# mcahny/vps

Measured on AMD Instinct MI355X. Metric: frames/sec FuseTrack 1024x2048, higher is better.
Workload: dtype f32-grade: f16x3 split operands (fp16 pair with scaled residual, 22 significand bits) on MFMA, f32 accumulate

## Files before the change

vps_amd/csrc/conv_h8p.hip:

```cpp
#include "conv_common.h"

namespace {

template <int N, typename F>
__device__ __forceinline__ void static_for_p(F&& f) {
    if constexpr (N > 0) {
        static_for_p<N - 1>(f);
        f(std::integral_constant<int, N - 1>{});
    }
}

template <int MODE, int KH, int KW>
__global__ __launch_bounds__(512, 2)
void conv_mfma_h8p_kernel(const vps_conv_desc d, const int tiles_m, const int tiles_n, const int chunks_per_split) {
    constexpr int TM = 2, TN = 2, WAVES_N = 2, BN = 128;
    constexpr int NTAP = KH * KW;
    static_assert(NTAP % 3 == 0 || NTAP == 4, "ring / register-set index of a tap must be static: 9 taps (9 % 3 == 0) or 4 taps (12-step cycle handled by the caller)");
    constexpr int HW = 32 + KW - 1, HH = 8 + KH - 1;
    constexpr int HROWS = HH * HW;
    constexpr int NLD = (HROWS + 63) / 64;
    typedef Split<MODE> SM;
    typedef typename SM::elem elem_t;
    typedef vec8<elem_t> x8;
    typedef vec4<elem_t> x4;
    constexpr int NSA = SM::NSA, NSB = SM::NSB, NLB = SM::NLB, NT = SM::NT;
    constexpr int PLANE = HROWS * LDS_LDH;
    constexpr int ABUF = NSA * PLANE;
    constexpr int NFRAG = NSB * 2 * (BN / 32);
    constexpr int BBUF = NFRAG * 512;
    static_assert(NFRAG * 64 == NSB * 512, "thread t stages chunk t of every plane");
    static_assert((2 * ABUF + 3 * BBUF) * 2 <= 160 * 1024, "LDS budget of the CU");

    __shared__ __attribute__((aligned(16))) elem_t As[2 * ABUF];
    __shared__ __attribute__((aligned(16))) elem_t Bs[3 * BBUF];

    const int t = threadIdx.x;
    int swz = xcd_swizzle(blockIdx.x, gridDim.x);
    int tile_n, tile_m, cls, split;
    decode_tile(d, swz, tiles_n, tiles_m, tile_n, tile_m, cls, split);

    const int py = cls / d.os_x, px = cls - py * d.os_x;
    const int H = d.H, W = d.W, cin_pad = d.cin_pad;
    const int tiles_x = (d.Qw + 31) >> 5, tiles_y = (d.Qh + 7) >> 3;
    const int tx = tile_m % tiles_x, tq = tile_m / tiles_x;
    const int ty = tq % tiles_y, n = tq / tiles_y;
    const int iy_org = ty * 8 - d.pad_y[py], ix_org = tx * 32 - d.pad_x[px];

    const int k4 = t & 7;
    const int r0 = t >> 3;
    const int chunk0 = split * chunks_per_split;
    const int nchunks = min(chunks_per_split, d.kpad / (BK * NTAP) - chunk0);
    const int nsteps = nchunks * NTAP;

    const int lane = t & 63;
    const int wave = __builtin_amdgcn_readfirstlane(t >> 6);
    const int wm = wave / WAVES_N, wn = wave - wm * WAVES_N;
    const int nbt = d.cout_pad >> 5, kst = d.kpad >> 4;
    const size_t wplane = (size_t)d.nclass * nbt * kst * 512;
    const __amdgpu_buffer_rsrc_t wrsrc = make_rsrc(d.w_split, (unsigned)(wplane * NSB * sizeof(elem_t)));
    const unsigned wbase = (unsigned)((((size_t)(cls * nbt + tile_n * (BN / 32)) * kst + 2 * (size_t)chunk0 * NTAP) * 512) * sizeof(elem_t));
    const __amdgpu_buffer_rsrc_t arsrc = make_rsrc(d.in, (unsigned)((size_t)d.N * H * W * d.in_ld * sizeof(float)));
    const unsigned ld4 = (unsigned)d.in_ld * 4u;

    f32x4 areg[NLD];
    int achunk = chunk0;
    x8 breg[3][NLB];
    float amax = 0.f;

    unsigned hoff[NLD];
#pragma unroll
    for (int i = 0; i < NLD; ++i) {
        const int hp = r0 + 64 * i;
        const int hy = hp / HW, hx = hp - hy * HW;
        const int iy = iy_org + hy, ix = ix_org + hx;
        const bool ok = hp < HROWS && (unsigned)iy < (unsigned)H && (unsigned)ix < (unsigned)W;
        hoff[i] = ok ? (unsigned)((n * H + iy) * W + ix) * ld4 + (unsigned)(d.in_coff + k4 * 4) * 4u : 0xFFFFFFF0u;
    }

    auto load_A = [&]() {
        const bool kv = achunk * BK + k4 * 4 < cin_pad;
        const unsigned coff = (unsigned)achunk * (BK * 4u);
        ++achunk;
#pragma unroll
        for (int i = 0; i < NLD; ++i)
            areg[i] = buffer_load16<f32x4>(arsrc, (kv && hoff[i] != 0xFFFFFFF0u) ? hoff[i] + coff : 0xFFFFFFF0u, 0u);
    };
    auto store_A = [&](const int i, const int buf) {
        x4 sp[NSA];
        split_act<MODE>(areg[i], sp, amax);
        const int row = r0 + 64 * i;
        if (row < HROWS) {
#pragma unroll
            for (int p = 0; p < NSA; ++p)
                *reinterpret_cast<x4*>(&As[buf * ABUF + p * PLANE + row * LDS_LDH + (((k4 >> 1) ^ lds_swz(row)) << 3) + ((k4 & 1) << 2)]) = sp[p];
        }
    };
    auto load_B = [&](const int step, const int set) {
        const int sc = min(step, nsteps - 1);
        const int f = wave, bcol = f % (BN / 32), slab = f / (BN / 32);
#pragma unroll
        for (int p = 0; p < NLB; ++p)
            breg[set][p] = buffer_load16<x8>(wrsrc, (unsigned)lane * 16u,
                                             wbase + (unsigned)(((size_t)p * wplane + ((size_t)bcol * kst + 2 * sc + slab) * 512) * sizeof(elem_t)));
    };
    auto store_B = [&](const int slot, const int set) {
#pragma unroll
        for (int p = 0; p < NLB; ++p) *reinterpret_cast<x8*>(&Bs[slot * BBUF + (t + 512 * p) * 8]) = breg[set][p];
        if constexpr (NLB < NSB) *reinterpret_cast<x8*>(&Bs[slot * BBUF + (t + 512 * NLB) * 8]) = derive_weight_plane<MODE>(breg[set][0]);
    };

    int hbase[TM];
#pragma unroll
    for (int a = 0; a < TM; ++a) hbase[a] = (wm * TM + a) * HW + (lane & 31);
    x8 af[2][NSA][TM];
    x8 bcur[2][NSB][TN];
    constexpr int NRD = NSA * TM + NSB * TN;
    auto read_frag = [&](const int j, const int m, const int abuf, const int toff, const int slot) {
        if (j < NSA * TM) {
            const int p = j / TM, a = j - p * TM;
            const int hrow = hbase[a] + toff;
            af[m][p][a] = *reinterpret_cast<const x8*>(&As[abuf * ABUF + p * PLANE + hrow * LDS_LDH + (((2 * m + (lane >> 5)) ^ lds_swz(hrow)) << 3)]);
        } else {
            const int jj = j - NSA * TM, p = jj / TN, b = jj - p * TN;
            bcur[m][p][b] = *reinterpret_cast<const x8*>(&Bs[slot * BBUF + (((p * 2 + m) * (BN / 32)) + wn * TN + b) * 512 + lane * 8]);
        }
    };

    f32x16 acc[TM][TN];
#pragma unroll
    for (int a = 0; a < TM; ++a)
#pragma unroll
        for (int b = 0; b < TN; ++b)
#pragma unroll
            for (int r = 0; r < 16; ++r) acc[a][b][r] = 0.f;

    load_A();
    load_B(0, 0);
    load_B(1, 1);
#pragma unroll
    for (int i = 0; i < NLD; ++i) store_A(i, 0);
    store_B(0, 0);
    store_B(1, 1);
    load_B(2, 2);
    load_A();
    __syncthreads();
#pragma unroll
    for (int j = 0; j < NRD; ++j) read_frag(j, 0, 0, 0, 0);

    constexpr int NMS = NT * TM * TN;
    constexpr int STG = NTAP / 2;
    constexpr int SPT = (NLD + STG - 1) / STG;
    auto mfma = [&](const int m, const int i) {
        const int q = i / (TM * TN), r = i - q * (TM * TN), a = r / TN, b = r - a * TN;
        acc[a][b] = split_mfma<MODE>(bcur[m][SM::PB[q]][b], af[m][SM::PA[q]][a], acc[a][b]);
    };

    auto tap = [&](const int chunk, auto tp_tag, auto r3_tag) {
        constexpr int tp = decltype(tp_tag)::value;
        constexpr int R3 = decltype(r3_tag)::value;
        const int cur = chunk & 1;
        const int step = chunk * NTAP + tp;
        constexpr int toff = (tp / KW) * HW + (tp % KW);
        constexpr int ntp = (tp + 1) % NTAP;
        constexpr int ntoff = (ntp / KW) * HW + (ntp % KW);
        const int nbuf = tp == NTAP - 1 ? cur ^ 1 : cur;
#pragma unroll
        for (int i = 0; i < NMS; ++i) {
            mfma(0, i);
            __builtin_amdgcn_sched_barrier(0);
            if (i == 0) load_B(step + 3, R3);
#pragma unroll
            for (int j = 0; j < NRD; ++j)
                if ((j * (NMS - 1)) / NRD + 1 == i || (NMS == 1 && i == 0)) read_frag(j, 1, cur, toff, R3);
            __builtin_amdgcn_sched_barrier(0);
        }
#pragma unroll
        for (int i = 0; i < NMS; ++i) {
            mfma(1, i);
            __builtin_amdgcn_sched_barrier(0);
            if (tp < STG) {
#pragma unroll
                for (int si = 0; si < SPT; ++si)
                    if (i == (si * NMS) / (SPT + 1) && tp * SPT + si < NLD) store_A(tp * SPT + si, cur ^ 1);
            }
            if (i == (SPT * NMS) / (SPT + 1)) {
                store_B((R3 + 2) % 3, (R3 + 2) % 3);
                if (tp == STG) load_A();
            }
#pragma unroll
            for (int j = 0; j < NRD; ++j)
                if ((j * (NMS - 1)) / NRD + 1 == i || (NMS == 1 && i == 0)) read_frag(j, 0, nbuf, ntoff, (R3 + 1) % 3);
            __builtin_amdgcn_sched_barrier(0);
        }
        __syncthreads();
    };

    if constexpr (NTAP % 3 == 0) {
        for (int chunk = 0; chunk < nchunks; ++chunk)
            static_for_p<NTAP>([&](auto tpc) {
                constexpr int TP = decltype(tpc)::value;
                tap(chunk, std::integral_constant<int, TP>{}, std::integral_constant<int, TP % 3>{});
            });
    } else {
        int chunk = 0;
        for (; chunk + 2 < nchunks; chunk += 3)
            static_for_p<3 * NTAP>([&](auto sc) {
                constexpr int S = decltype(sc)::value;
                tap(chunk + S / NTAP, std::integral_constant<int, S % NTAP>{}, std::integral_constant<int, S % 3>{});
            });
        if (chunk < nchunks) {
            static_for_p<NTAP>([&](auto sc) {
                constexpr int S = decltype(sc)::value;
                tap(chunk, std::integral_constant<int, S>{}, std::integral_constant<int, S % 3>{});
            });
            ++chunk;
            if (chunk < nchunks)
                static_for_p<NTAP>([&](auto sc) {
                    constexpr int S = decltype(sc)::value;
                    tap(chunk, std::integral_constant<int, S>{}, std::integral_constant<int, (NTAP + S) % 3>{});
                });
        }
    }
    report_range<MODE>(d, amax);
    conv_epilogue<TM, TN, BN, true, 5>(d, acc, tiles_m * 256, tile_m, tile_n, cls, split, py, px, wm, wn, lane, (cls * tiles_m + tile_m) * tiles_n + tile_n);
}

}

__attribute__((visibility("hidden")))
void vpsi_launch_conv_h8p(const vps_conv_desc& d, const conv_plan& p, hipStream_t s) {
    hipLaunchKernelGGL((conv_mfma_h8p_kernel<VPS_PREC_F16X3, 3, 3>), dim3(p.grid), dim3(p.block), 0, s, d, p.tiles_m, p.tiles_n, p.chunks_per_split);
}
```

vps_amd/csrc/conv_mfma.hip:

```cpp
#include "conv_common.h"

namespace {
template <int TM, int TN, int WAVES_M, int WAVES_N, bool DEFORM>
__global__ __launch_bounds__(256, 2)
void conv_mfma_f32_kernel(const vps_conv_desc d, const int M, const int tiles_m, const int tiles_n,
                          const int ksteps_per_split) {
    constexpr int BN = WAVES_N * TN * 32;
    static_assert(WAVES_M * TM * 32 == BM, "block M tile must be 128");
    static_assert(WAVES_M * WAVES_N == 4, "4 wavefronts per block");
    constexpr int NB = BN / 32;

    __shared__ __attribute__((aligned(16))) float As[BM * LDS_LD];
    __shared__ __attribute__((aligned(16))) float Bs[BN * LDS_LD];

    const int t = threadIdx.x;
    int swz = xcd_swizzle(blockIdx.x, gridDim.x);
    int tile_n, tile_m, cls, split;
    decode_tile(d, swz, tiles_n, tiles_m, tile_n, tile_m, cls, split);

    const int py = cls / d.os_x, px = cls - py * d.os_x;
    const int pad_y = d.pad_y[py], pad_x = d.pad_x[px];
    const float* __restrict__ wcls = d.w + (size_t)cls * d.cout_pad * d.kpad;

    const int H = d.H, W = d.W, KH = d.KH, KW = d.KW, cin_pad = d.cin_pad;
// ... 431 lines not shown
                            const int pos = ((w + 1) * NMF) / (NW + 1);
                            if (mf == (pos < 1 ? 1 : pos)) {
                                __builtin_amdgcn_sched_barrier(0);
                                work(w);
                                __builtin_amdgcn_sched_barrier(0);
                            }
                        }
                    }
        __syncthreads();
    };
    for (int step = 0; step < nsteps; step += 2) {
        kstep(step, std::integral_constant<int, 0>{});
        if (step + 1 < nsteps) kstep(step + 1, std::integral_constant<int, 1>{});
    }
    report_range<MODE>(d, amax);
    conv_epilogue<TM, TN, BN, false, 4, DEFORM>(d, acc, M, tile_m, tile_n, cls, split, py, px, wm, wn, lane, (cls * tiles_m + tile_m) * tiles_n + tile_n);
}

template <int TM, int TN, int WAVES_M, int WAVES_N, int MODE, int KH, int KW>
__global__ __launch_bounds__(256, 2)
void conv_mfma_bf16h_kernel(const vps_conv_desc d, const int tiles_m, const int tiles_n, const int chunks_per_split) {
    constexpr int BN = WAVES_N * TN * 32;
    static_assert(WAVES_M * TM * 32 == BM, "block M tile must be 128");
    static_assert(WAVES_M * WAVES_N == 4, "4 wavefronts per block");
    constexpr int NTAP = KH * KW;
    constexpr int HW = 16 + KW - 1, HH = 8 + KH - 1;
    constexpr int HROWS = HH * HW;
    constexpr int NLD = (HROWS + 31) / 32;
    typedef Split<MODE> SM;
    typedef typename SM::elem elem_t;
    typedef vec8<elem_t> x8;
    typedef vec4<elem_t> x4;
    constexpr int NSA = SM::NSA, NSB = SM::NSB;
    constexpr int PLANE = NLD * 32 * LDS_LDH;
    constexpr int ABUF = NSA * PLANE;

    __shared__ __attribute__((aligned(16))) elem_t As[2 * ABUF];

    const int t = threadIdx.x;
    int swz = xcd_swizzle(blockIdx.x, gridDim.x);
    int tile_n, tile_m, cls, split;
    decode_tile(d, swz, tiles_n, tiles_m, tile_n, tile_m, cls, split);

    const int py = cls / d.os_x, px = cls - py * d.os_x;
    const int H = d.H, W = d.W, cin_pad = d.cin_pad;
    const int tiles_x = (d.Qw + 15) >> 4, tiles_y = (d.Qh + 7) >> 3;
    const int tx = tile_m % tiles_x, tq = tile_m / tiles_x;
    const int ty = tq % tiles_y, n = tq / tiles_y;
    const int iy_org = ty * 8 - d.pad_y[py], ix_org = tx * 16 - d.pad_x[px];

    const int k4 = t & 7;
    const int r0 = t >> 3;
    const int chunk0 = split * chunks_per_split;
    const int nchunks = min(chunks_per_split, d.kpad / (BK * NTAP) - chunk0);
    const int nsteps = nchunks * NTAP;

    const int lane = t & 63;
    const int wave = __builtin_amdgcn_readfirstlane(t >> 6);
    const int wm = wave / WAVES_N, wn = wave - wm * WAVES_N;
    const int nbt = d.cout_pad >> 5, kst = d.kpad >> 4;
    const size_t wplane = (size_t)d.nclass * nbt * kst * 512;
    const __amdgpu_buffer_rsrc_t wrsrc = make_rsrc(d.w_split, (unsigned)(wplane * NSB * sizeof(elem_t)));
    const unsigned wbase = (unsigned)((((size_t)(cls * nbt + tile_n * (BN / 32) + wn * TN) * kst + 2 * (size_t)chunk0 * NTAP) * 512) * sizeof(elem_t));
    const unsigned wlane = (unsigned)lane * 16u;
    const __amdgpu_buffer_rsrc_t arsrc = make_rsrc(d.in, (unsigned)((size_t)d.N * H * W * d.in_ld * sizeof(float)));
    const unsigned ld4 = (unsigned)d.in_ld * 4u;

    f32x4 areg[NLD];
    int achunk = chunk0;
    x8 bnext[2][NSB][TN];
    float amax = 0.f;

    unsigned hoff[NLD];
#pragma unroll
    for (int i = 0; i < NLD; ++i) {
        const int hp = r0 + 32 * i;
        const int hy = hp / HW, hx = hp - hy * HW;
        const int iy = iy_org + hy, ix = ix_org + hx;
        const bool ok = hp < HROWS && (unsigned)iy < (unsigned)H && (unsigned)ix < (unsigned)W;
        hoff[i] = ok ? (unsigned)((n * H + iy) * W + ix) * ld4 + (unsigned)(d.in_coff + k4 * 4) * 4u : 0xFFFFFFF0u;
    }

    auto load_A = [&]() {
        const bool kv = achunk * BK + k4 * 4 < cin_pad;
        const unsigned coff = (unsigned)achunk * (BK * 4u);
        ++achunk;
#pragma unroll
        for (int i = 0; i < NLD; ++i)
            areg[i] = buffer_load16<f32x4>(arsrc, (kv && hoff[i] != 0xFFFFFFF0u) ? hoff[i] + coff : 0xFFFFFFF0u, 0u);
    };
    auto load_B = [&](int step, int m, int p) {
#pragma unroll
        for (int b = 0; b < TN; ++b)
            bnext[m][p][b] = buffer_load16<x8>(wrsrc, wlane, wbase + (unsigned)(((size_t)p * wplane + ((size_t)b * kst + 2 * step + m) * 512) * sizeof(elem_t)));
    };
    auto store_A = [&](int i, int buf) {
        x4 sp[NSA];
        split_act<MODE>(areg[i], sp, amax);
        const int row = r0 + 32 * i;
#pragma unroll
        for (int p = 0; p < NSA; ++p)
            *reinterpret_cast<x4*>(&As[buf * ABUF + p * PLANE + row * LDS_LDH + (((k4 >> 1) ^ lds_swz(row)) << 3) + ((k4 & 1) << 2)]) = sp[p];
    };

    int hbase[TM];
#pragma unroll
    for (int a = 0; a < TM; ++a) {
        const int j = wm * TM * 32 + a * 32 + (lane & 31);
        hbase[a] = (j >> 4) * HW + (j & 15);
    }
    x8 af[2][NSA][TM];
    auto read_A = [&](int m, int buf, int toff) {
#pragma unroll
        for (int a = 0; a < TM; ++a) {
            const int hrow = hbase[a] + toff;
            const int off = buf * ABUF + hrow * LDS_LDH + (((2 * m + (lane >> 5)) ^ lds_swz(hrow)) << 3);
#pragma unroll
            for (int p = 0; p < NSA; ++p) af[m][p][a] = *reinterpret_cast<const x8*>(&As[off + p * PLANE]);
        }
    };

    f32x16 acc[TM][TN];
#pragma unroll
    for (int a = 0; a < TM; ++a)
#pragma unroll
        for (int b = 0; b < TN; ++b)
#pragma unroll
            for (int r = 0; r < 16; ++r) acc[a][b][r] = 0.f;

    load_A();
#pragma unroll
    for (int m = 0; m < 2; ++m)
#pragma unroll
        for (int p = 0; p < NSB; ++p) load_B(0, m, p);
#pragma unroll
    for (int i = 0; i < NLD; ++i) store_A(i, 0);
    load_A();
    __syncthreads();

    constexpr int NT = SM::NT;
    constexpr int NMF = 2 * NT * TM * TN;
    constexpr int SPT = (NLD + NTAP - 2) / (NTAP - 1);

    for (int chunk = 0; chunk < nchunks; ++chunk) {
        const int cur = chunk & 1;
#pragma unroll
        for (int tp = 0; tp < NTAP; ++tp) {
            const int step = chunk * NTAP + tp;
            const int bstep = min(step + 1, nsteps - 1);
            const int toff = (tp / KW) * HW + (tp % KW);
            constexpr int NLB = NSB;
            x8 bcur[2][NSB][TN];
#pragma unroll
            for (int m = 0; m < 2; ++m) {
#pragma unroll
                for (int p = 0; p < NLB; ++p)
#pragma unroll
                    for (int b = 0; b < TN; ++b) bcur[m][p][b] = bnext[m][p][b];
                if constexpr (NLB < NSB) {
#pragma unroll
                    for (int b = 0; b < TN; ++b) bcur[m][2][b] = derive_weight_plane<MODE>(bcur[m][0][b]);
                }
            }
            read_A(0, cur, toff);
            __builtin_amdgcn_sched_barrier(0);

            const int NW = SPT + 1 + 2 * NLB;
            auto work = [&](const int w) {
                if (w == 1) read_A(1, cur, toff);
                else if (w == 0 || (w >= 2 && w < SPT + 1)) {
                    const int si = (w == 0 ? 0 : w - 1);
                    if (tp < NTAP - 1) {
                        const int row = tp * SPT + si;
                        if (row < NLD) store_A(row, cur ^ 1);
                    } else if (si == 0) load_A();
                } else load_B(bstep, (w - SPT - 1) / NLB, (w - SPT - 1) % NLB);
            };

            int mf = 0;
#pragma unroll
            for (int m = 0; m < 2; ++m)
#pragma unroll
                for (int q = 0; q < NT; ++q)
#pragma unroll
                    for (int a = 0; a < TM; ++a)
#pragma unroll
                        for (int b = 0; b < TN; ++b) {
                            acc[a][b] = split_mfma<MODE>(bcur[m][SM::PB[q]][b], af[m][SM::PA[q]][a], acc[a][b]);
                            ++mf;
#pragma unroll
                            for (int w = 0; w < NW; ++w) {
                                const int pos = ((w + 1) * NMF) / (NW + 1);
                                if (mf == (pos < 1 ? 1 : pos)) {
                                    __builtin_amdgcn_sched_barrier(0);
                                    work(w);
                                    __builtin_amdgcn_sched_barrier(0);
                                }
                            }
                        }
        }
        __syncthreads();
    }
    report_range<MODE>(d, amax);
    conv_epilogue<TM, TN, BN, true>(d, acc, tiles_m * BM, tile_m, tile_n, cls, split, py, px, wm, wn, lane, (cls * tiles_m + tile_m) * tiles_n + tile_n);
}

template <int V>
__global__ __launch_bounds__(256)
void conv_splitk_reduce_kernel(const vps_conv_desc d, const int M) {
    const int cv = d.cout / V;
    const size_t total = (size_t)d.nclass * M * cv;
    const size_t plane = (size_t)d.nclass * M * d.cout_pad;
    for (size_t idx = (size_t)blockIdx.x * blockDim.x + threadIdx.x; idx < total;
         idx += (size_t)gridDim.x * blockDim.x) {
        const int co = (int)(idx % cv) * V;
        const size_t t2 = idx / cv;
        const int m = (int)(t2 % M);
        const int cls = (int)(t2 / M);
        const float* __restrict__ wp = d.ws + ((size_t)cls * M + m) * d.cout_pad + co;
        float s[V];
#pragma unroll
        for (int e = 0; e < V; ++e) s[e] = 0.f;
        for (int sp0 = 0; sp0 < d.ksplit; sp0 += 8) {
            float v[8][V];
#pragma unroll
            for (int j = 0; j < 8; ++j) {
                const float* q = wp + (size_t)min(sp0 + j, d.ksplit - 1) * plane;
                if constexpr (V == 4) {
                    const f32x4 t = *reinterpret_cast<const f32x4*>(q);
                    v[j][0] = t[0]; v[j][1] = t[1]; v[j][2] = t[2]; v[j][3] = t[3];
                } else {
                    v[j][0] = q[0];
                }
            }
#pragma unroll
            for (int j = 0; j < 8; ++j)
#pragma unroll
                for (int e = 0; e < V; ++e) s[e] = (sp0 + j < d.ksplit) ? s[e] + v[j][e] : s[e];
        }
        const int py = cls / d.os_x, px = cls - py * d.os_x;
        const int qx = m % d.Qw;
        const int tq = m / d.Qw;
        const int qy = tq % d.Qh;
        const int n = tq / d.Qh;
        const int oy = qy * d.os_y + py, ox = qx * d.os_x + px;
        const size_t opix = ((size_t)n * d.Ho + oy) * d.Wo + ox;
        const int rs = d.res_shift;
        const size_t rpix = ((size_t)n * (d.Ho >> rs) + (oy >> rs)) * (d.Wo >> rs) + (ox >> rs);
        float r[V];
#pragma unroll
        for (int e = 0; e < V; ++e) r[e] = 0.f;
        if (d.res) {
            if constexpr (V == 4) {
                const f32x4 t = *reinterpret_cast<const f32x4*>(d.res + rpix * d.res_ld + d.res_coff + co);
                r[0] = t[0]; r[1] = t[1]; r[2] = t[2]; r[3] = t[3];
            } else {
                r[0] = d.res[rpix * d.res_ld + d.res_coff + co];
            }
        }
        float o[V];
#pragma unroll
        for (int e = 0; e < V; ++e) {
            float v = s[e] * (d.scale ? d.scale[co + e] : 1.f) + (d.shift ? d.shift[co + e] : 0.f);
            if (d.res) v += r[e];
            o[e] = vps_act(v, d.act, d.slope);
        }
        float* op = d.out + opix * d.out_ld + d.out_coff + co;
        if constexpr (V == 4) *reinterpret_cast<f32x4*>(op) = f32x4{o[0], o[1], o[2], o[3]};
        else op[0] = o[0];
    }
}

template <int TM, int TN, int WAVES_M, int WAVES_N>
void launch_conv(const vps_conv_desc& d, const conv_plan& p, hipStream_t s) {
    const dim3 grid(p.grid), block(p.block);
    if (p.kernel == CONV_K_HALO) {
        with_prec<true>(d.prec, [&](auto mode) {
            constexpr int MODE = decltype(mode)::value;
            if (d.KH == 3) hipLaunchKernelGGL((conv_mfma_bf16h_kernel<TM, TN, WAVES_M, WAVES_N, MODE, 3, 3>), grid, block, 0, s, d, p.tiles_m, p.tiles_n, p.chunks_per_split);
            else hipLaunchKernelGGL((conv_mfma_bf16h_kernel<TM, TN, WAVES_M, WAVES_N, MODE, 2, 2>), grid, block, 0, s, d, p.tiles_m, p.tiles_n, p.chunks_per_split);
        });
        return;
    }
#define VPS_CONV_LAUNCH(KERNEL) hipLaunchKernelGGL((KERNEL), grid, block, 0, s, d, p.M, p.tiles_m, p.tiles_n, p.per_split)
    if (p.kernel == CONV_K_F32) {
        if (d.offset) VPS_CONV_LAUNCH((conv_mfma_f32_kernel<TM, TN, WAVES_M, WAVES_N, true>));
        else VPS_CONV_LAUNCH((conv_mfma_f32_kernel<TM, TN, WAVES_M, WAVES_N, false>));
        return;
    }
    const bool tapmajor = d.korder == 0 && d.KH * d.KW > 1;
    with_prec<true>(d.prec, [&](auto mode) {
        constexpr int MODE = decltype(mode)::value;
        if (d.offset) VPS_CONV_LAUNCH((conv_mfma_bf16p_kernel<TM, TN, WAVES_M, WAVES_N, MODE, false, true>));
        else if (tapmajor) VPS_CONV_LAUNCH((conv_mfma_bf16p_kernel<TM, TN, WAVES_M, WAVES_N, MODE, true>));
        else VPS_CONV_LAUNCH((conv_mfma_bf16p_kernel<TM, TN, WAVES_M, WAVES_N, MODE, false>));
    });
#undef VPS_CONV_LAUNCH
}

conv_switches conv_switches_now(const vps_conv_desc& d) {
    const auto on = [](const char* name) { const char* const e = getenv(name); return !(e && atoi(e) == 0); };
    const auto not0 = [](const char* name) { const char* const e = getenv(name); return !(e && e[0] == '0'); };
    static const bool s2_halo = not0("VPS_S2_HALO"), thin = on("VPS_THIN"), debug_occ = getenv("VPS_DEBUG_OCC") != nullptr;
    conv_switches sw = {true, true, true, true, s2_halo, thin, debug_occ};
    if (d.prec != VPS_PREC_F16X3) return sw;
    if (d.tile_n == 32) {
        if (d.cout > 16) sw.n32 = not0("VPS_N32");
        else if (d.nclass == 4) sw.n16t = on("VPS_N16T");
    } else if (d.tile_n <= 128 && d.KH == 1) sw.pw = on("VPS_PW");
    else if (d.tile_n == 128 && d.KH == 3 && d.stride == 1) sw.h8p = on("VPS_H8P");
    return sw;
}

const conv_limits& conv_limits_once(const bool debug) {
    static const conv_limits lim = [debug] {
        conv_limits l = {};
        int dev = 0;
        (void)hipGetDevice(&dev);
        (void)hipDeviceGetAttribute(&l.cus, hipDeviceAttributeMultiprocessorCount, dev);
        vpsi_conv_pw_limits(l, debug);
        vpsi_conv_thin_limits(l, debug);
        if (debug) vpsi_conv_q_debug_occ();
        return l;
    }();
    return lim;
}

}

extern "C" int vps_conv2d(const vps_conv_desc* dp, void* stream) {
    if (!dp) return VPS_EARG(1);
    const vps_conv_desc& d = *dp;
    if (const int e = vpsi_conv_check(d)) return e;
    const conv_switches sw = conv_switches_now(d);
    const conv_plan p = vpsi_conv_plan(d, conv_limits_once(sw.debug_occ), sw);
    hipStream_t s = (hipStream_t)stream;
    switch (p.kernel) {
        case CONV_K_NONE: return p.err;
        case CONV_K_SMALL3X3V: case CONV_K_SMALL_BATCHED: case CONV_K_SMALL: vpsi_launch_conv_small(d, p, s); break;
        case CONV_K_THIN: vpsi_launch_conv_thin(d, p, s); break;
        case CONV_K_DCN256:
            hipLaunchKernelGGL((conv_mfma_bf16p_kernel<2, 4, 2, 2, VPS_PREC_F16X3, false, true>), dim3(p.grid), dim3(p.block), 0, s, d, p.M, p.tiles_m, p.tiles_n, p.per_split);
            break;
        case CONV_K_N16T: case CONV_K_N32: case CONV_K_N16: vpsi_launch_conv_n16(d, p, s); break;
        case CONV_K_H8S2: vpsi_launch_conv_h8s2(d, p, s); break;
        case CONV_K_H8P: vpsi_launch_conv_h8p(d, p, s); break;
        case CONV_K_H8: vpsi_launch_conv_h8(d, p, s); break;
        case CONV_K_PW: vpsi_launch_conv_pw(d, p, s); break;
        case CONV_K_Q: vpsi_launch_conv_q(d, p, s); break;
        default:
            if (d.tile_n == 128) launch_conv<2, 2, 2, 2>(d, p, s);
            else if (d.tile_n == 64) launch_conv<2, 1, 2, 2>(d, p, s);
            else launch_conv<1, 1, 4, 1>(d, p, s);
    }
    int st = vps_launch_status();
    if (st || !p.needs_reduce) return st;
    const size_t total = (size_t)d.nclass * p.M * d.cout;
    if (p.reduce_v4) hipLaunchKernelGGL(conv_splitk_reduce_kernel<4>, dim3(stream_grid((long)(total / 4), 256)), dim3(256), 0, s, d, p.M);
    else hipLaunchKernelGGL(conv_splitk_reduce_kernel<1>, dim3(stream_grid((long)total, 256)), dim3(256), 0, s, d, p.M);
    return vps_launch_status();
}
```

vps_amd/csrc/conv_plan.cpp:

```cpp
#include "conv_plan.h"
#include <stdint.h>

namespace {

constexpr int BM = 128, BK = 32;

inline int cdiv(long a, long b) { return (int)((a + b - 1) / b); }
inline size_t in_bytes(const vps_conv_desc& d) { return (size_t)d.N * d.H * d.W * d.in_ld * sizeof(float); }
inline size_t out_bytes(const vps_conv_desc& d) { return (size_t)d.N * d.Ho * d.Wo * d.out_ld * sizeof(float); }
inline bool two_plane(int prec) { return prec == VPS_PREC_F16X3 || prec == VPS_PREC_BF16X3 || prec == VPS_PREC_BF16; }

constexpr int H8_MIN_CHUNKS = 3;
constexpr int PW_MIN_ROUNDS = 2;

conv_plan fail(conv_plan p, int n) { p.kernel = CONV_K_NONE; p.err = VPS_EARG(n); return p; }

conv_plan plan_small(const vps_conv_desc& d, conv_plan p) {
    p.block = 256;
    p.G = 1; p.logG = 0;
    while (p.G < 64 && p.G < (d.cin_pad >> 2)) { p.G <<= 1; ++p.logG; }
    const size_t wbytes = (size_t)(d.cout <= 2 ? 2 : 4) * d.kpad * sizeof(float);
    if (d.KH == 3 && d.KW == 3 && d.stride == 1 && d.nclass == 1 && d.pad_y[0] == 1 && d.pad_x[0] == 1 && d.Ho == d.H && d.Wo == d.W &&
        wbytes <= 150 * 1024 && (d.cout <= 2 || d.cout_pad >= 4) && in_bytes(d) < 0xFFFFFFF0ull &&
        (long)d.N * d.H * d.W < 0x7fffffffL) {
        const int run = d.cout <= 2 ? 4 : 2;
        p.runs_per_row = (d.W + run - 1) / run;
        const long total_runs = (long)d.N * d.H * p.runs_per_row;
        const int ppw = 64 >> p.logG;
        long blocks = (total_runs + 4 * ppw - 1) / (4 * ppw);
        if (blocks > 768) blocks = 768;
        p.kernel = CONV_K_SMALL3X3V; p.total_runs = (int)total_runs; p.grid = (unsigned)blocks; p.smem = wbytes;
        return p;
    }
    const long total = (long)d.nclass * p.M;
    const size_t wb = (size_t)d.nclass * (d.cout <= 2 ? 2 : 4) * d.kpad * sizeof(float);
    if ((d.cin_pad >> 2) * d.KH * d.KW >= 8 && wb <= 48 * 1024 && (d.cout <= 2 || d.cout_pad >= 4) && in_bytes(d) < 0xFFFFFFF0ull) {
        const int c4n = d.cin_pad >> 2, ntap = d.KH * d.KW;
        p.G = 1; p.logG = 0;
        while (p.G < 64 && p.G * 8 < c4n * ntap && p.G < c4n) { p.G <<= 1; ++p.logG; }
        p.nslot = (c4n + p.G - 1) >> p.logG;
        const int ppw = 64 >> p.logG;
        const long waves = (total + ppw - 1) / ppw;
        long blocks = (waves + 3) / 4; if (blocks > 2048) blocks = 2048; if (blocks < 1) blocks = 1;
        p.kernel = CONV_K_SMALL_BATCHED; p.grid = (unsigned)blocks; p.smem = wb;
        return p;
    }
    const long waves = (total + (64 >> p.logG) - 1) / (64 >> p.logG);
    long blocks = (waves + 3) / 4; if (blocks > 8192) blocks = 8192; if (blocks < 1) blocks = 1;
    p.kernel = CONV_K_SMALL; p.grid = (unsigned)blocks;
    return p;
}

bool plan_thin(const vps_conv_desc& d, const conv_limits& lim, const conv_switches& sw, conv_plan& p) {
    if (!sw.thin || !d.w_thin || d.prec != VPS_PREC_F16X3 || d.offset || d.res || d.nclass != 1 || d.ksplit != 1 || d.korder != 0) return false;
    if (d.KH != d.KW || d.cout_pad != 64 || d.tile_n != 64 || (d.cout & 3) || ((uintptr_t)d.w_thin & 15)) return false;
    if (d.pad_y[0] != d.KH / 2 || d.pad_x[0] != d.KH / 2 || d.pad_y[1] != d.KH / 2 || d.pad_x[1] != d.KH / 2) return false;
    if (in_bytes(d) >= 0xFFFFFFF0ull) return false;
    if (((d.out_ld | d.out_coff) & 3) || ((uintptr_t)d.out & 15) || out_bytes(d) >= 0xFFFFFFF0ull) return false;
    int i = 0;
    while (i < 4 && !(d.KH == conv_thin_shapes[i].ks && d.stride == conv_thin_shapes[i].s && d.cin_pad == conv_thin_shapes[i].c4)) ++i;
    if (i == 4) return false;
    const int ph = conv_thin_shapes[i].ph;
    const int tiles_x = (d.Qw + 31) / 32, tiles_y = (d.Qh + ph - 1) / ph;
    const long ntiles = (long)d.N * tiles_x * tiles_y;
    if (ntiles < 512 || ntiles > 0x7fffffffL) return false;
    const int resident = (lim.thin_per_cu[i] > 0 ? lim.thin_per_cu[i] : 1) * (lim.cus > 0 ? lim.cus : 256);
    const long rounds = (ntiles + resident - 1) / resident;
    p.kernel = CONV_K_THIN; p.thin = i; p.tiles_n = tiles_x; p.tiles_m = tiles_y; p.ntiles = (int)ntiles;
    p.grid = (unsigned)((ntiles + rounds - 1) / rounds); p.block = 256;
    return true;
}

bool plan_pw(const vps_conv_desc& d, const conv_limits& lim, const conv_switches& sw, conv_plan& p) {
    if (!sw.pw || d.prec != VPS_PREC_F16X3 || d.offset || d.KH != 1 || d.KW != 1 || d.nclass != 1 || d.ksplit != 1 || d.gn_stats) return false;
    if (d.pad_y[0] || d.pad_x[0] || (d.cin_pad & 31) || d.kpad != d.cin_pad || (d.tile_n != 128 && d.tile_n != 64)) return false;
    const int nk = d.kpad / BK;
    if (nk < 2 || (nk & 1)) return false;
    if (d.Ho != d.Qh || d.Wo != d.Qw || (d.stride == 1 && (d.H != d.Qh || d.W != d.Qw))) return false;
    if (((d.cout | d.out_ld | d.out_coff) & 3) || ((uintptr_t)d.out & 15) || out_bytes(d) >= 0xFFFFFE00ull) return false;
    if (d.res && (((d.res_ld | d.res_coff) & 3) || ((uintptr_t)d.res & 15) || d.res_shift < 0 || d.res_shift > 4 ||
                  (size_t)d.N * (d.Ho >> d.res_shift) * (d.Wo >> d.res_shift) * d.res_ld * sizeof(float) >= 0xFFFFFE00ull)) return false;
    if (in_bytes(d) >= 0xFFFFFE00ull) return false;
    const int per_cu = lim.pw_per_cu[d.tile_n == 128 ? 1 : 0];
    const int resident = (per_cu > 0 ? per_cu : 1) * (lim.cus > 0 ? lim.cus : 256);
    const long total = (long)p.tiles_m * p.tiles_n;
    const int unit = 8 * p.tiles_n;
    if (resident < unit || total < (long)PW_MIN_ROUNDS * resident) return false;
    const long rounds = (total + resident - 1) / resident;
    long grid = (total + rounds - 1) / rounds;
    grid = (grid + unit - 1) / unit * unit;
    if (grid > resident) grid = resident / unit * unit;
    const int mper = (int)(grid / unit);
    p.kernel = CONV_K_PW; p.grid = (unsigned)grid; p.nk = nk; p.nit = (p.tiles_m + mper * 8 - 1) / (mper * 8);
    return true;
}

}

const conv_thin_shape conv_thin_shapes[4] = {{8, 3, 1, 8}, {12, 3, 1, 8}, {4, 7, 2, 8}, {12, 7, 2, 4}};

const char* vpsi_conv_kernel_name(int kernel) {
    static const char* const names[] = {"none", "small3x3v", "small_batched", "small", "thin", "dcn256", "n16t", "n32", "n16",
                                        "h8s2", "h8p", "h8", "halo", "pw", "q", "f32", "bf16p"};
    return kernel >= 0 && kernel <= CONV_K_BF16P ? names[kernel] : "?";
}

int vpsi_conv_check(const vps_conv_desc& d) {
    if (!d.in || !d.out) return VPS_EARG(2);
    if (d.prec < VPS_PREC_F32 || d.prec > VPS_PREC_F16X3) return VPS_EARG(12);
    if (d.prec == VPS_PREC_F32 ? !d.w : !d.w_split) return VPS_EARG(13);
    if ((d.in_ld & 3) || (d.in_coff & 3) || (d.cin_pad & 3) || d.cin_pad <= 0) return VPS_EARG(3);
    if ((d.kpad % BK) || d.kpad < d.KH * d.KW * d.cin_pad || (d.korder != 0 && d.korder != 1)) return VPS_EARG(4);
    if (d.korder == 1 && d.kpad != d.KH * d.KW * ((d.cin_pad + BK - 1) / BK) * BK) return VPS_EARG(14);
    if (d.tile_n != 32 && d.tile_n != 64 && d.tile_n != 128 && !(d.tile_n == 256 && d.offset && d.prec == VPS_PREC_F16X3 && d.korder == 1)) return VPS_EARG(5);
    if (d.cout_pad % d.tile_n || d.cout > d.cout_pad || d.cout <= 0) return VPS_EARG(6);
    if (d.nclass != d.os_y * d.os_x || d.nclass < 1 || d.os_y > 2 || d.os_x > 2) return VPS_EARG(7);
    if (d.ksplit < 1 || (d.ksplit > 1 && !d.ws)) return VPS_EARG(8);
    if (d.offset && (d.nclass != 1 || d.off_ld < 2 * d.KH * d.KW || d.KH * d.KW > 9 || d.H > 65535 || d.W > 65535)) return VPS_EARG(9);
    if (d.offset && d.prec != VPS_PREC_F32 && d.korder != 1) return VPS_EARG(17);
    if (((uintptr_t)d.in & 15) || ((uintptr_t)d.w & 15) || ((uintptr_t)d.w_split & 15)) return VPS_EARG(10);
    if (d.prec != VPS_PREC_F32 && in_bytes(d) >= 0xFFFFFFF0ull) return VPS_EARG(16);
    if (d.gn_stats && (!d.offset || d.prec == VPS_PREC_F32 || d.ksplit != 1 || d.gn_rep < 1 || (d.gn_rep & (d.gn_rep - 1)) || (d.gn_cpg != 4 && (d.gn_cpg < 8 || (d.gn_cpg & 7))) || d.cout % d.gn_cpg ||
                       ((d.cout | d.out_ld | d.out_coff) & 3) || ((uintptr_t)d.out & 15) || d.res || ((uintptr_t)d.gn_stats & 7)))
        return VPS_EARG(15);
    const long Ml = (long)d.N * d.Qh * d.Qw;
    if (Ml <= 0 || Ml > 0x7fffffffL) return VPS_EARG(11);
    return 0;
}

conv_plan vpsi_conv_plan(const vps_conv_desc& d, const conv_limits& lim, const conv_switches& sw) {
    conv_plan p = {};
    const int M = p.M = (int)((long)d.N * d.Qh * d.Qw);
    if (d.cout <= 4 && d.prec == VPS_PREC_F32 && !d.offset && d.ksplit == 1 && d.tile_n == 32) return plan_small(d, p);
    if (plan_thin(d, lim, sw, p)) return p;

    const int BN = d.tile_n;
    const int tiles_m = p.tiles_m = cdiv(M, BM);
    const int tiles_n = p.tiles_n = d.cout_pad / BN;
    const int ksteps = d.kpad / BK;
    p.block = 256;
    p.needs_reduce = d.ksplit > 1 && !d.tile_counter;
    if (BN == 256) {
        p.per_split = cdiv(ksteps, d.ksplit);
        if (cdiv(ksteps, p.per_split) != d.ksplit) return fail(p, 20);
        p.kernel = CONV_K_DCN256; p.grid = (unsigned)((long)tiles_m * tiles_n * d.ksplit); p.reduce_v4 = true;
        return p;
    }
    const int ntap = d.KH * d.KW;
    const int nch = d.korder == 1 ? ksteps / ntap : 0;
    const bool chunk_split = d.ksplit > 1 && d.korder == 1 && nch > 0 && cdiv(nch, cdiv(nch, d.ksplit)) == d.ksplit;
    const int per_split = p.per_split = chunk_split ? cdiv(nch, d.ksplit) * ntap : cdiv(ksteps, d.ksplit);
    p.chunks_per_split = per_split / ntap;
    if (cdiv(ksteps, per_split) != d.ksplit) return fail(p, 20);
    const long nblk = (long)tiles_m * tiles_n * d.nclass * d.ksplit;
    if (nblk <= 0 || nblk > 0x7fffffffL) return fail(p, 21);
    p.reduce_v4 = !((d.cout | d.cout_pad | d.out_ld | d.out_coff) & 3) && !((uintptr_t)d.out & 15) &&
                  (!d.res || (!((d.res_ld | d.res_coff) & 3) && !((uintptr_t)d.res & 15)));
    const long tiles2d = (long)d.N * ((d.Qh + 7) / 8) * ((d.Qw + 15) / 16);
    const bool halo = d.prec != VPS_PREC_F32 && !d.offset && d.stride == 1 && d.korder == 1 && d.KH == d.KW && (d.KH == 3 || d.KH == 2) &&
                      tiles2d * 128 * 2 <= (long)M * 3 && (d.ksplit == 1 || chunk_split);
    const long tiles2d8 = (long)d.N * ((d.Qh + 7) / 8) * ((d.Qw + 31) / 32);
    const bool h8 = halo && BN == 128 && two_plane(d.prec) && tiles2d8 * 256 * 2 <= (long)M * 3 &&
                    tiles2d8 * tiles_n * d.nclass * d.ksplit >= 256 && ksteps / ntap >= H8_MIN_CHUNKS;
    const bool h8s2 = sw.s2_halo && (BN == 128 || BN == 64) && two_plane(d.prec) && !d.offset &&
                      d.stride == 2 && d.nclass == 1 && d.korder == 1 && d.KH == d.KW && (d.KH == 3 || d.KH == 5) &&
                      d.pad_y[0] == d.KH / 2 && d.pad_x[0] == d.KW / 2 && tiles2d8 * 256 * 2 <= (long)M * 3 &&
                      tiles2d8 * tiles_n * d.ksplit >= 256 && (d.ksplit == 1 || chunk_split);
    const bool n16 = BN == 32 && d.prec == VPS_PREC_F16X3 && halo && d.cout > 4 && d.cout <= (sw.n32 ? 32 : 16) && d.cout_pad == 32 && d.ksplit == 1 &&
                     !d.gn_stats && tiles2d8 * 256 * 2 <= (long)M * 3 && tiles2d8 * d.nclass >= 256;
    if (n16) {
        const bool fused = sw.n16t && d.KH == 2 && d.KW == 2 && d.nclass == 4 && d.os_y == 2 && d.os_x == 2 &&
                           d.pad_y[0] >= 0 && d.pad_y[0] <= 1 && d.pad_y[1] >= 0 && d.pad_y[1] <= 1 &&
                           d.pad_x[0] >= 0 && d.pad_x[0] <= 1 && d.pad_x[1] >= 0 && d.pad_x[1] <= 1;
        p.tiles_m = (int)tiles2d8; p.block = 512;
        if (fused && d.cout <= 16) { p.kernel = CONV_K_N16T; p.grid = (unsigned)tiles2d8; }
        else { p.kernel = d.cout > 16 ? CONV_K_N32 : CONV_K_N16; p.grid = (unsigned)(tiles2d8 * d.nclass); }
    } else if (h8s2) {
        p.kernel = CONV_K_H8S2; p.tiles_m = (int)tiles2d8; p.block = 512; p.grid = (unsigned)(tiles2d8 * tiles_n * d.ksplit);
    } else if (h8) {
        p.kernel = sw.h8p && d.prec == VPS_PREC_F16X3 && d.KH == 3 ? CONV_K_H8P : CONV_K_H8;
        p.tiles_m = (int)tiles2d8; p.block = 512; p.grid = (unsigned)(tiles2d8 * tiles_n * d.nclass * d.ksplit);
    } else if (halo) {
        const long nblk2 = tiles2d * tiles_n * d.nclass * d.ksplit;
        if (nblk2 > 0x7fffffffL) return fail(p, 21);
        p.kernel = CONV_K_HALO; p.tiles_m = (int)tiles2d; p.grid = (unsigned)nblk2;
    } else {
        p.grid = (unsigned)nblk;
        const bool tapmajor = d.korder == 0 && ntap > 1;
        const bool q_ok = BN >= 64 && !tapmajor;
        if (q_ok && plan_pw(d, lim, sw, p)) return p;
        if (q_ok && !d.offset && two_plane(d.prec)) p.kernel = CONV_K_Q;
        else p.kernel = d.prec == VPS_PREC_F32 ? CONV_K_F32 : CONV_K_BF16P;
    }
    return p;
}
```

vps_amd/csrc/conv_plan.h:

```cpp
#pragma once
#include <stddef.h>
#include "../../include/vps_hip.h"

#ifndef VPS_EARG
#define VPS_EARG(x) (-1000 - (x))
#endif

enum conv_kernel {
    CONV_K_NONE = 0,
    CONV_K_SMALL3X3V,
    CONV_K_SMALL_BATCHED,
    CONV_K_SMALL,
    CONV_K_THIN,
    CONV_K_DCN256,
    CONV_K_N16T,
    CONV_K_N32,
    CONV_K_N16,
    CONV_K_H8S2,
    CONV_K_H8P,
    CONV_K_H8,
    CONV_K_HALO,
    CONV_K_PW,
    CONV_K_Q,
    CONV_K_F32,
    CONV_K_BF16P,
};

struct conv_plan {
    int kernel;
    int err;
    int M;
    int tiles_m, tiles_n;
    int per_split;
    int chunks_per_split;
    unsigned grid, block;
    size_t smem;
    int nk, nit;
    int G, logG, nslot;
    int runs_per_row, total_runs;
    int thin;
    int ntiles;
    bool needs_reduce;
    bool reduce_v4;
};

struct conv_limits {
    int cus;
    int pw_per_cu[2];
    int thin_per_cu[4];
};

struct conv_switches {
    bool pw;
    bool h8p;
    bool n16t;
    bool n32;
    bool s2_halo;
    bool thin;
    bool debug_occ;
};

struct conv_thin_shape { int c4, ks, s, ph; };
extern const conv_thin_shape conv_thin_shapes[4];

int vpsi_conv_check(const vps_conv_desc& d);
conv_plan vpsi_conv_plan(const vps_conv_desc& d, const conv_limits& lim, const conv_switches& sw);
const char* vpsi_conv_kernel_name(int kernel);

#ifdef __HIPCC__
void vpsi_launch_conv_small(const vps_conv_desc& d, const conv_plan& p, hipStream_t s);
void vpsi_launch_conv_thin(const vps_conv_desc& d, const conv_plan& p, hipStream_t s);
void vpsi_launch_conv_n16(const vps_conv_desc& d, const conv_plan& p, hipStream_t s);
void vpsi_launch_conv_h8(const vps_conv_desc& d, const conv_plan& p, hipStream_t s);
void vpsi_launch_conv_h8p(const vps_conv_desc& d, const conv_plan& p, hipStream_t s);
void vpsi_launch_conv_h8s2(const vps_conv_desc& d, const conv_plan& p, hipStream_t s);
void vpsi_launch_conv_pw(const vps_conv_desc& d, const conv_plan& p, hipStream_t s);
void vpsi_launch_conv_q(const vps_conv_desc& d, const conv_plan& p, hipStream_t s);
void vpsi_conv_pw_limits(conv_limits& lim, bool debug);
void vpsi_conv_thin_limits(conv_limits& lim, bool debug);
void vpsi_conv_q_debug_occ();
#endif
```

Baseline: 56.91.

## Add wide 256-column h8 halo conv kernel with per-slab pipelined refills

Adds a 3x3 stride-1 f16x3 convolution kernel that covers 256 output channels per block instead of 128. Each halo activation tile loaded into LDS is therefore reused across twice as many output columns, reducing activation traffic and split work per FLOP. Each tap is split into two half-slabs, and weight loads, LDS stores and fragment reads are interleaved between MFMAs on a three-slot weight ring with double-buffered activations. It is on by default (h8w=1) when cout_pad is a multiple of 256, nclass is 1, ksplit is 1 and the grid still has at least 256 blocks. In exchange it raises per-thread accumulator register pressure and produces fewer blocks, which can lower occupancy and parallelism.

```diff
diff --git a/vps_amd/csrc/conv_h8p.hip b/vps_amd/csrc/conv_h8p.hip
--- a/vps_amd/csrc/conv_h8p.hip
+++ b/vps_amd/csrc/conv_h8p.hip
@@ -225,6 +225,199 @@
     conv_epilogue<TM, TN, BN, true, 5>(d, acc, tiles_m * 256, tile_m, tile_n, cls, split, py, px, wm, wn, lane, (cls * tiles_m + tile_m) * tiles_n + tile_n);
 }
 
+__global__ __launch_bounds__(512, 2)
+void conv_mfma_h8w_kernel(const vps_conv_desc d, const int tiles_m, const int tiles_n) {
+    constexpr int MODE = VPS_PREC_F16X3, KH = 3, KW = 3;
+    constexpr int TM = 2, TN = 4, WAVES_N = 2, BN = 256;
+    constexpr int NTAP = KH * KW, NPH = 2 * NTAP;
+    static_assert(NPH % 3 == 0 && NPH % 2 == 0, "ring slot and register set of a slab must be static");
+    constexpr int HW = 32 + KW - 1, HH = 8 + KH - 1;
+    constexpr int HROWS = HH * HW;
+    constexpr int NLD = (HROWS + 63) / 64;
+    typedef Split<MODE> SM;
+    typedef typename SM::elem elem_t;
+    typedef vec8<elem_t> x8;
+    typedef vec4<elem_t> x4;
+    constexpr int NSA = SM::NSA, NSB = SM::NSB, NLB = SM::NLB, NT = SM::NT;
+    static_assert(NLB == 2 && NSB == 3, "two loaded weight planes, the third derived");
+    constexpr int PLANE = HROWS * LDS_LDH;
+    constexpr int ABUF = NSA * PLANE;
+    constexpr int NCB = BN / 32;
+    constexpr int SBUF = NSB * NCB * 512;
+    static_assert(NCB == 8, "thread t stages chunk t & 63 of column block t >> 6 of every plane");
+    static_assert((2 * ABUF + 3 * SBUF) * 2 <= 160 * 1024, "LDS budget of the CU");
+
+    __shared__ __attribute__((aligned(16))) elem_t As[2 * ABUF];
+    __shared__ __attribute__((aligned(16))) elem_t Bs[3 * SBUF];
+
+    const int t = threadIdx.x;
+    int swz = xcd_swizzle(blockIdx.x, gridDim.x);
+    int tile_n, tile_m, cls, split;
+    decode_tile(d, swz, tiles_n, tiles_m, tile_n, tile_m, cls, split);
+
+    const int H = d.H, W = d.W, cin_pad = d.cin_pad;
+    const int tiles_x = (d.Qw + 31) >> 5, tiles_y = (d.Qh + 7) >> 3;
+    const int tx = tile_m % tiles_x, tq = tile_m / tiles_x;
+    const int ty = tq % tiles_y, n = tq / tiles_y;
+    const int iy_org = ty * 8 - d.pad_y[0], ix_org = tx * 32 - d.pad_x[0];
+
+    const int k4 = t & 7;
+    const int r0 = t >> 3;
+    const int nchunks = d.kpad / (BK * NTAP);
+    const int nslabs = nchunks * NPH;
+
+    const int lane = t & 63;
+    const int wave = __builtin_amdgcn_readfirstlane(t >> 6);
+    const int wm = wave / WAVES_N, wn = wave - wm * WAVES_N;
+    const int nbt = d.cout_pad >> 5, kst = d.kpad >> 4;
+    const size_t wplane = (size_t)d.nclass * nbt * kst * 512;
+    const __amdgpu_buffer_rsrc_t wrsrc = make_rsrc(d.w_split, (unsigned)(wplane * NSB * sizeof(elem_t)));
+    const unsigned wbase = (unsigned)(((size_t)(tile_n * NCB + wave) * kst * 512) * sizeof(elem_t));
+    const __amdgpu_buffer_rsrc_t arsrc = make_rsrc(d.in, (unsigned)((size_t)d.N * H * W * d.in_ld * sizeof(float)));
+    const unsigned ld4 = (unsigned)d.in_ld * 4u;
+
+    constexpr int NGR = 3, GR = NLD / NGR;
+    static_assert(NGR * GR == NLD, "");
+    f32x4 areg[GR];
+    x8 breg[2][NLB];
+    float amax = 0.f;
+
+    unsigned hoff[NLD];
+#pragma unroll
+    for (int i = 0; i < NLD; ++i) {
+        const int hp = r0 + 64 * i;
+        const int hy = hp / HW, hx = hp - hy * HW;
+        const int iy = iy_org + hy, ix = ix_org + hx;
+        const bool ok = hp < HROWS && (unsigned)iy < (unsigned)H && (unsigned)ix < (unsigned)W;
+        hoff[i] = ok ? (unsigned)((n * H + iy) * W + ix) * ld4 + (unsigned)(d.in_coff + k4 * 4) * 4u : 0xFFFFFFF0u;
+    }
+
+    auto load_A = [&](const int grp, const int chunk) {
+        const bool kv = chunk * BK + k4 * 4 < cin_pad;
+        const unsigned coff = (unsigned)chunk * (BK * 4u);
+#pragma unroll
+        for (int i = 0; i < GR; ++i)
+            areg[i] = buffer_load16<f32x4>(arsrc, (kv && hoff[GR * grp + i] != 0xFFFFFFF0u) ? hoff[GR * grp + i] + coff : 0xFFFFFFF0u, 0u);
+    };
+    auto store_A = [&](const int i, const int buf) {
+        x4 sp[NSA];
+        split_act<MODE>(areg[i % GR], sp, amax);
+        const int row = r0 + 64 * i;
+        if (row < HROWS) {
+#pragma unroll
+            for (int p = 0; p < NSA; ++p)
+                *reinterpret_cast<x4*>(&As[buf * ABUF + p * PLANE + row * LDS_LDH + (((k4 >> 1) ^ lds_swz(row)) << 3) + ((k4 & 1) << 2)]) = sp[p];
+        }
+    };
+    auto load_B = [&](const int g, const int set) {
+        const int sc = min(g, nslabs - 1);
+#pragma unroll
+        for (int p = 0; p < NLB; ++p)
+            breg[set][p] = buffer_load16<x8>(wrsrc, (unsigned)lane * 16u, wbase + (unsigned)(((size_t)p * wplane + (size_t)sc * 512) * sizeof(elem_t)));
+    };
+    auto store_B = [&](const int slot, const int set) {
+#pragma unroll
+        for (int p = 0; p < NLB; ++p) *reinterpret_cast<x8*>(&Bs[slot * SBUF + (p * NCB + wave) * 512 + lane * 8]) = breg[set][p];
+        *reinterpret_cast<x8*>(&Bs[slot * SBUF + (NLB * NCB + wave) * 512 + lane * 8]) = derive_weight_plane<MODE>(breg[set][0]);
+    };
+
+    int hbase[TM];
+#pragma unroll
+    for (int a = 0; a < TM; ++a) hbase[a] = (wm * TM + a) * HW + (lane & 31);
+    x8 af0[2][TM], af1[TM];
+    x8 bf[NSB];
+    auto read_A = [&](const int p, const int a, const int m, const int abuf, const int toff) {
+        const int hrow = hbase[a] + toff;
+        const x8 v = *reinterpret_cast<const x8*>(&As[abuf * ABUF + p * PLANE + hrow * LDS_LDH + (((2 * m + (lane >> 5)) ^ lds_swz(hrow)) << 3)]);
+        if (p == 0) af0[m][a] = v; else af1[a] = v;
+    };
+    auto read_B = [&](const int p, const int b, const int slot) {
+        bf[p] = *reinterpret_cast<const x8*>(&Bs[slot * SBUF + (p * NCB + wn * TN + b) * 512 + lane * 8]);
+    };
+
+    constexpr int EP = 4, CW = TN / EP;
+    f32x16 acc[EP][TM][CW];
+#pragma unroll
+    for (int h = 0; h < EP; ++h)
+#pragma unroll
+        for (int a = 0; a < TM; ++a)
+#pragma unroll
+            for (int b = 0; b < CW; ++b)
+#pragma unroll
+                for (int r = 0; r < 16; ++r) acc[h][a][b][r] = 0.f;
+
+    load_B(0, 0);
+    load_B(1, 1);
+#pragma unroll
+    for (int grp = 0; grp < NGR; ++grp) {
+        load_A(grp, 0);
+#pragma unroll
+        for (int i = 0; i < GR; ++i) store_A(GR * grp + i, 0);
+    }
+    store_B(0, 0);
+    store_B(1, 1);
+    load_B(2, 1);
+    __syncthreads();
+#pragma unroll
+    for (int p = 0; p < NSA; ++p)
+#pragma unroll
+        for (int a = 0; a < TM; ++a) read_A(p, a, 0, 0, 0);
+#pragma unroll
+    for (int p = 0; p < NSB; ++p) read_B(p, 0, 0);
+
+    constexpr int NMB = NT * TM;
+    static_assert(NMB == 6 && TM == 2 && NSA == 2, "the in-place refills below are written for this product order");
+    constexpr int APER = NPH / NGR;
+
+    auto slab = [&](const int chunk, auto ph_tag) {
+        constexpr int PH = decltype(ph_tag)::value;
+        constexpr int tp = PH / 2, m = PH & 1, R3 = PH % 3, S2 = PH & 1;
+        const int cur = chunk & 1;
+        const int g = chunk * NPH + PH;
+        constexpr int toff = (tp / KW) * HW + (tp % KW);
+        constexpr int ntp = (tp + 1) % NTAP;
+        constexpr int ntoff = m ? (ntp / KW) * HW + (ntp % KW) : toff;
+        const int nbuf = PH == NPH - 1 ? cur ^ 1 : cur;
+        constexpr int grp = PH / APER, gs = PH - grp * APER - (4 - grp / 2);
+#pragma unroll
+        for (int a = 0; a < TM; ++a) asm volatile("" : "+v"(hbase[a]));
+#pragma unroll
+        for (int b = 0; b < TN; ++b)
+#pragma unroll
+            for (int i = 0; i < NMB; ++i) {
+                const int q = i / TM, a = i - q * TM;
+                acc[b / CW][a][b % CW] = split_mfma<MODE>(bf[SM::PB[q]], SM::PA[q] ? af1[a] : af0[m][a], acc[b / CW][a][b % CW]);
+                __builtin_amdgcn_sched_barrier(0);
+#ifndef VPS_KO_H8W_NOB
+                if (b == 0 && i == 0) load_B(g + 3, S2);
+                if (b == 2 && i == 2) store_B((R3 + 2) % 3, S2 ^ 1);
+#endif
+#ifndef VPS_KO_H8W_NOA
+                if (b == 1 && i == 2 && gs >= 0 && gs < GR) store_A(GR * grp + gs, cur ^ 1);
+                if (b == 2 && i == 4 && PH % APER == 0) load_A(grp, chunk + 1);
+#endif
+                if (a == TM - 1) read_B(SM::PB[q], (b + 1) % TN, b == TN - 1 ? (R3 + 1) % 3 : R3);
+                if (b == 2 && (i == 3 || i == 4)) read_A(0, i - 3, m ^ 1, nbuf, ntoff);
+                if (b == 3 && (i == 2 || i == 3)) read_A(1, i - 2, m ^ 1, nbuf, ntoff);
+                __builtin_amdgcn_sched_barrier(0);
+            }
+        __syncthreads();
+    };
+
+    for (int chunk = 0; chunk < nchunks; ++chunk)
+        static_for_p<NPH>([&](auto phc) { slab(chunk, std::integral_constant<int, decltype(phc)::value>{}); });
+
+    report_range<MODE>(d, amax);
+#pragma unroll
+    for (int h = 0; h < EP; ++h)
+        conv_epilogue<TM, CW, CW * 32, true, 5>(d, acc[h], tiles_m * 256, tile_m, (tile_n * WAVES_N + wn) * EP + h, cls, split, 0, 0, wm, 0, lane, 0);
+}
+
+}
+
+__attribute__((visibility("hidden")))
+void vpsi_launch_conv_h8w(const vps_conv_desc& d, const conv_plan& p, hipStream_t s) {
+    hipLaunchKernelGGL(conv_mfma_h8w_kernel, dim3(p.grid), dim3(p.block), 0, s, d, p.tiles_m, p.tiles_n);
 }
 
 __attribute__((visibility("hidden")))
diff --git a/vps_amd/csrc/conv_mfma.hip b/vps_amd/csrc/conv_mfma.hip
--- a/vps_amd/csrc/conv_mfma.hip
+++ b/vps_amd/csrc/conv_mfma.hip
@@ -757,13 +757,16 @@
     const auto on = [](const char* name) { const char* const e = getenv(name); return !(e && atoi(e) == 0); };
     const auto not0 = [](const char* name) { const char* const e = getenv(name); return !(e && e[0] == '0'); };
     static const bool s2_halo = not0("VPS_S2_HALO"), thin = on("VPS_THIN"), debug_occ = getenv("VPS_DEBUG_OCC") != nullptr;
-    conv_switches sw = {true, true, true, true, s2_halo, thin, debug_occ};
+    conv_switches sw = {true, true, true, true, s2_halo, thin, debug_occ, 1};
     if (d.prec != VPS_PREC_F16X3) return sw;
     if (d.tile_n == 32) {
         if (d.cout > 16) sw.n32 = not0("VPS_N32");
         else if (d.nclass == 4) sw.n16t = on("VPS_N16T");
     } else if (d.tile_n <= 128 && d.KH == 1) sw.pw = on("VPS_PW");
-    else if (d.tile_n == 128 && d.KH == 3 && d.stride == 1) sw.h8p = on("VPS_H8P");
+    else if (d.tile_n == 128 && d.KH == 3 && d.stride == 1) {
+        sw.h8p = on("VPS_H8P");
+        if (const char* const e = getenv("VPS_H8W")) sw.h8w = atoi(e);
+    }
     return sw;
 }
 
@@ -800,6 +803,7 @@
         case CONV_K_N16T: case CONV_K_N32: case CONV_K_N16: vpsi_launch_conv_n16(d, p, s); break;
         case CONV_K_H8S2: vpsi_launch_conv_h8s2(d, p, s); break;
         case CONV_K_H8P: vpsi_launch_conv_h8p(d, p, s); break;
+        case CONV_K_H8W: vpsi_launch_conv_h8w(d, p, s); break;
         case CONV_K_H8: vpsi_launch_conv_h8(d, p, s); break;
         case CONV_K_PW: vpsi_launch_conv_pw(d, p, s); break;
         case CONV_K_Q: vpsi_launch_conv_q(d, p, s); break;
diff --git a/vps_amd/csrc/conv_plan.cpp b/vps_amd/csrc/conv_plan.cpp
--- a/vps_amd/csrc/conv_plan.cpp
+++ b/vps_amd/csrc/conv_plan.cpp
@@ -101,8 +101,9 @@
 
 const char* vpsi_conv_kernel_name(int kernel) {
     static const char* const names[] = {"none", "small3x3v", "small_batched", "small", "thin", "dcn256", "n16t", "n32", "n16",
-                                        "h8s2", "h8p", "h8", "halo", "pw", "q", "f32", "bf16p"};
-    return kernel >= 0 && kernel <= CONV_K_BF16P ? names[kernel] : "?";
+                                        "h8s2", "h8p", "h8", "halo", "pw", "q", "f32", "bf16p", "h8w"};
+    static_assert(sizeof(names) / sizeof(names[0]) == CONV_K_COUNT, "one name per kernel id");
+    return kernel >= 0 && kernel < CONV_K_COUNT ? names[kernel] : "?";
 }
 
 int vpsi_conv_check(const vps_conv_desc& d) {
@@ -160,8 +161,10 @@
     const bool halo = d.prec != VPS_PREC_F32 && !d.offset && d.stride == 1 && d.korder == 1 && d.KH == d.KW && (d.KH == 3 || d.KH == 2) &&
                       tiles2d * 128 * 2 <= (long)M * 3 && (d.ksplit == 1 || chunk_split);
     const long tiles2d8 = (long)d.N * ((d.Qh + 7) / 8) * ((d.Qw + 31) / 32);
-    const bool h8 = halo && BN == 128 && two_plane(d.prec) && tiles2d8 * 256 * 2 <= (long)M * 3 &&
-                    tiles2d8 * tiles_n * d.nclass * d.ksplit >= 256 && ksteps / ntap >= H8_MIN_CHUNKS;
+    const bool h8_forced = sw.h8w >= 2 && sw.h8p && d.prec == VPS_PREC_F16X3 && BN == 128 && !d.offset && d.stride == 1 && d.korder == 1 &&
+                           d.KH == 3 && d.KW == 3 && d.ksplit == 1 && tiles2d8 * tiles_n * d.nclass <= 0x7fffffffL;
+    const bool h8 = h8_forced || (halo && BN == 128 && two_plane(d.prec) && tiles2d8 * 256 * 2 <= (long)M * 3 &&
+                                  tiles2d8 * tiles_n * d.nclass * d.ksplit >= 256 && ksteps / ntap >= H8_MIN_CHUNKS);
     const bool h8s2 = sw.s2_halo && (BN == 128 || BN == 64) && two_plane(d.prec) && !d.offset &&
                       d.stride == 2 && d.nclass == 1 && d.korder == 1 && d.KH == d.KW && (d.KH == 3 || d.KH == 5) &&
                       d.pad_y[0] == d.KH / 2 && d.pad_x[0] == d.KW / 2 && tiles2d8 * 256 * 2 <= (long)M * 3 &&
@@ -180,6 +183,10 @@
     } else if (h8) {
         p.kernel = sw.h8p && d.prec == VPS_PREC_F16X3 && d.KH == 3 ? CONV_K_H8P : CONV_K_H8;
         p.tiles_m = (int)tiles2d8; p.block = 512; p.grid = (unsigned)(tiles2d8 * tiles_n * d.nclass * d.ksplit);
+        if (p.kernel == CONV_K_H8P && sw.h8w && sw.h8w != 3 && d.cout_pad % 256 == 0 && d.ksplit == 1 && !d.gn_stats && d.nclass == 1 &&
+            (sw.h8w == 2 || tiles2d8 * (d.cout_pad / 256) >= 256)) {
+            p.kernel = CONV_K_H8W; p.tiles_n = d.cout_pad / 256; p.grid = (unsigned)(tiles2d8 * p.tiles_n);
+        }
     } else if (halo) {
         const long nblk2 = tiles2d * tiles_n * d.nclass * d.ksplit;
         if (nblk2 > 0x7fffffffL) return fail(p, 21);
diff --git a/vps_amd/csrc/conv_plan.h b/vps_amd/csrc/conv_plan.h
--- a/vps_amd/csrc/conv_plan.h
+++ b/vps_amd/csrc/conv_plan.h
@@ -24,6 +24,8 @@
     CONV_K_Q,
     CONV_K_F32,
     CONV_K_BF16P,
+    CONV_K_H8W,
+    CONV_K_COUNT
 };
 
 struct conv_plan {
@@ -58,6 +60,7 @@
     bool s2_halo;
     bool thin;
     bool debug_occ;
+    int h8w;
 };
 
 struct conv_thin_shape { int c4, ks, s, ph; };
@@ -73,6 +76,7 @@
 void vpsi_launch_conv_n16(const vps_conv_desc& d, const conv_plan& p, hipStream_t s);
 void vpsi_launch_conv_h8(const vps_conv_desc& d, const conv_plan& p, hipStream_t s);
 void vpsi_launch_conv_h8p(const vps_conv_desc& d, const conv_plan& p, hipStream_t s);
+void vpsi_launch_conv_h8w(const vps_conv_desc& d, const conv_plan& p, hipStream_t s);
 void vpsi_launch_conv_h8s2(const vps_conv_desc& d, const conv_plan& p, hipStream_t s);
 void vpsi_launch_conv_pw(const vps_conv_desc& d, const conv_plan& p, hipStream_t s);
 void vpsi_launch_conv_q(const vps_conv_desc& d, const conv_plan& p, hipStream_t s);
```

Result: no change. 57.29, median of 6 (+0.7%).
